# simochen/flowtrack.pytorch

Hardware: AMD Instinct MI355X
Metric: pose crops/sec (ResNet-50 + 3-deconv head, 256x192) (higher is better)
Workload: dtype fp16; 1 GPU; ResNet-50 pose head fp16, batch 64 x 256x192 synthetic crops per GPU (BASELINE.json configs[1]); per_gpu_batch=64, resident_batches=4, parallelism=dp1: batch sharded, one process per GPU

## Files before the change

flowtrack/pytorch_amd/csrc/conv_direct.hip:

```cpp
#include <stdlib.h>

#include <type_traits>

#include "ft_common.h"
#include "conv_wstat.h"

namespace ft {
namespace {

struct CdParams {
  const char* x;
  const char* x2;
  const char* res;
  char* y;
  const char* ws;
  const float* scale;
  const float* shift;
  int M;
  int nc1, nc2;
  int x_cstride, x_coff;
  int HqWq, Wq;
  int x2_hi, x2_wi, x2_cstride, x2_coff, x2_stride;
  int y_cstride, y_coff, res_cstride, res_coff;
  int Cout, act;
  float slope;
  int npt, ncb;
  unsigned x_bytes, x2_bytes, y_bytes, res_bytes, ws_bytes;
  int cpt, kw, Hi, Wi, stride, pad;
  int dbg;
  int wmajor;
};

static inline int cd_wmajor(long long x_bytes, long long w_bytes, int npt, int ncb) {
  static const int mode = dev_env_int("FT_CD_WMAJOR", 0);
  if (mode != 2) return mode == 1;
  if (ncb < 8 || npt < 2) return 0;
  return 8 * x_bytes + w_bytes < x_bytes + 8 * w_bytes;
}

template <int N, int I = 0, typename F>
__device__ __forceinline__ void cd_unroll(F&& f) {
  if constexpr (I < N) {
    f(std::integral_constant<int, I>{});
    cd_unroll<N, I + 1>(f);
  }
}

#define CD_BARRIER() asm volatile("s_barrier" ::: "memory")

__host__ __device__ constexpr int cd_sigma(int r) { return 16 * ((r >> 2) & 1) + 4 * (r >> 3) + (r & 3); }

template <int CPR>
__device__ __forceinline__ int cd_key(int row) { return CPR < 16 ? ((row >> 1) & (CPR - 1)) : (row & 15); }

#ifndef FT_CD_WSLOTS
#define FT_CD_WSLOTS 3
#endif
template <int KSPLIT>
struct CdGeom {
  static constexpr int MT = 3, BP = 96;
  static constexpr int BN = KSPLIT == 1 ? 256 : 64;
  static constexpr int CHUNK_K = KSPLIT == 1 ? 64 : 256;
  static constexpr int ROWB = CHUNK_K * 2;
  static constexpr int XB = BP * ROWB;
  static constexpr int LX = XB / 1024 / 4;
  static constexpr int WCHUNK = 4 * 8 * 1024;
  static constexpr int STG_ROWB = BN * 2;
  static constexpr int RING = 3 * XB;
  static constexpr int PART = KSPLIT == 1 ? 0 : 4 * 6 * 4096;
  static constexpr int LDS_BYTES = (RING > PART + BP * STG_ROWB ? RING : PART + BP * STG_ROWB) + 2 * BN * 4;
  static_assert(LDS_BYTES <= 163840, "LDS map");
};

template <int KSPLIT, bool HAS_RES, int NCH, bool TAPS = false>
__global__ __launch_bounds__(256, 1) void conv_direct_kernel(const CdParams p) {
#if defined(__HIP_DEVICE_COMPILE__)
  using G = CdGeom<KSPLIT>;
  constexpr int MT = G::MT, BP = G::BP, BN = G::BN, ROWB = G::ROWB, XB = G::XB, LX = G::LX;
  constexpr int TAB = G::LDS_BYTES - 2 * BN * 4;
  extern __shared__ __attribute__((aligned(16))) char smem[];
  typedef __attribute__((address_space(3))) void* lds_ptr;
  using c0 = std::integral_constant<int, 0>;
  using c1 = std::integral_constant<int, 1>;
  using c2 = std::integral_constant<int, 2>;
  const int tid = threadIdx.x, lane = tid & 63;
  const int wave = __builtin_amdgcn_readfirstlane(tid >> 6);
  const int l31 = lane & 31, lhi = lane >> 5;

  int logical;
  {
    const int total = p.npt * p.ncb;
    const int b = blockIdx.x;
    const int q = total >> 3, r = total & 7, xcd = b & 7, loc = b >> 3;
    logical = (xcd < r ? xcd * (q + 1) : r * (q + 1) + (xcd - r) * q) + loc;
  }
  const int cb = p.wmajor ? logical / p.npt : logical % p.ncb, pt = p.wmajor ? logical % p.npt : logical / p.ncb;
  const int m0 = pt * BP;
  const int nchunk = NCH > 0 ? NCH : p.nc1 + p.nc2;

  const __amdgpu_buffer_rsrc_t rsrc_x = __builtin_amdgcn_make_buffer_rsrc(const_cast<char*>(p.x), 0, p.x_bytes, 0x00020000);
  const __amdgpu_buffer_rsrc_t rsrc_x2 = __builtin_amdgcn_make_buffer_rsrc(const_cast<char*>(p.nc2 ? p.x2 : p.x), 0, p.nc2 ? p.x2_bytes : p.x_bytes, 0x00020000);
  const __amdgpu_buffer_rsrc_t rsrc_y = __builtin_amdgcn_make_buffer_rsrc(p.y, 0, p.y_bytes, 0x00020000);
  const __amdgpu_buffer_rsrc_t rsrc_w = __builtin_amdgcn_make_buffer_rsrc(const_cast<char*>(p.ws), 0, p.ws_bytes, 0x00020000);
  constexpr unsigned kOOB = 0x80000000u;

  constexpr int CPR = ROWB / 16;
  constexpr int RPL = 64 / CPR;
  unsigned x_voff[LX], x2_voff[TAPS ? 1 : LX];
  int x_tmask[TAPS ? LX : 1];
#pragma unroll
  for (int t = 0; t < LX; ++t) {
    const int row = (t * 4 + wave) * RPL + lane / CPR, pos = lane % CPR;
    const int m = m0 + row;
    const unsigned swz = (unsigned)((pos ^ cd_key<CPR>(row)) << 4);
    unsigned v = kOOB, v2 = kOOB;
    if constexpr (TAPS) {
      int mk = 0;
      if (m < p.M) {
        const int n = m / p.HqWq, rem = m - n * p.HqWq, oy = rem / p.Wq, ox = rem - oy * p.Wq;
        const int iy0 = oy * p.stride - p.pad, ix0 = ox * p.stride - p.pad;
        v = (unsigned)((((n * p.Hi + iy0) * p.Wi + ix0) * p.x_cstride + p.x_coff) * 2) + swz;
        const int ntap = p.nc1 / p.cpt;
        for (int tp = 0; tp < ntap; ++tp) {
          const int ky = tp / p.kw, kx = tp - ky * p.kw;
          if ((unsigned)(iy0 + ky) < (unsigned)p.Hi && (unsigned)(ix0 + kx) < (unsigned)p.Wi) mk |= 1 << tp;
        }
      }
      x_tmask[t] = mk;
      x_voff[t] = v;
      continue;
    }
    if (m < p.M) {
      v = (unsigned)((m * p.x_cstride + p.x_coff) * 2) + swz;
      if (p.nc2) {
        const int n = m / p.HqWq, rem = m - n * p.HqWq, qy = rem / p.Wq, qx = rem - qy * p.Wq;
        v2 = (unsigned)((((n * p.x2_hi + qy * p.x2_stride) * p.x2_wi + qx * p.x2_stride) * p.x2_cstride + p.x2_coff) * 2) + swz;
      }
    }
    x_voff[t] = v;
    x2_voff[TAPS ? 0 : t] = v2;
  }
  auto issue_x = [&](int c, int buf) {
    char* dst = smem + buf * XB;
    if constexpr (TAPS) {
      const int tap = c / p.cpt, cc = c - tap * p.cpt;
      const int ky = tap / p.kw, kx = tap - ky * p.kw;
      const unsigned delta = (unsigned)(((ky * p.Wi + kx) * p.x_cstride) * 2 + cc * ROWB);
#pragma unroll
      for (int t = 0; t < LX; ++t)
        __builtin_amdgcn_raw_ptr_buffer_load_lds(rsrc_x, (lds_ptr)(dst + (t * 4 + wave) * 1024), 16,
                                                 ((x_tmask[t] >> tap) & 1) ? x_voff[t] + delta : kOOB, 0, 0, 0);
    } else if (c < p.nc1) {
#pragma unroll
      for (int t = 0; t < LX; ++t)
        __builtin_amdgcn_raw_ptr_buffer_load_lds(rsrc_x, (lds_ptr)(dst + (t * 4 + wave) * 1024), 16, x_voff[t], c * ROWB, 0, 0);
    } else {
#pragma unroll
      for (int t = 0; t < LX; ++t)
        __builtin_amdgcn_raw_ptr_buffer_load_lds(rsrc_x2, (lds_ptr)(dst + (t * 4 + wave) * 1024), 16, x2_voff[t], (c - p.nc1) * ROWB, 0, 0);
    }
  };
  const unsigned lane16 = (unsigned)lane * 16u;
  constexpr int WS = NCH > 0 ? FT_CD_WSLOTS : 3;
  uint4_t areg[WS][4][2];
  auto load_a = [&](auto slotc, int c) {
    constexpr int SL = decltype(slotc)::value;
    const int base = c < nchunk ? ((cb * nchunk + c) * 4 + wave) * 8192 : 0x7fff0000;
#pragma unroll
    for (int kk = 0; kk < 4; ++kk)
#pragma unroll
      for (int i = 0; i < 2; ++i)
        areg[SL][kk][i] = __builtin_amdgcn_raw_buffer_load_b128(rsrc_w, lane16, base + (kk * 2 + i) * 1024, 0);
  };

  if (tid < BN / 4) {
    const float4_t one = {1.f, 1.f, 1.f, 1.f}, zero = {0.f, 0.f, 0.f, 0.f};
    const int ch = cb * BN + tid * 4;
    reinterpret_cast<float4_t*>(smem + TAB)[tid] = p.scale ? *reinterpret_cast<const float4_t*>(p.scale + ch) : one;
    reinterpret_cast<float4_t*>(smem + TAB + BN * 4)[tid] = p.shift ? *reinterpret_cast<const float4_t*>(p.shift + ch) : zero;
  }
  constexpr int NTILE = 2 * MT;
  const int wtile0 = KSPLIT == 1 ? 2 * wave : 0;
  uint4_t rres[HAS_RES ? (KSPLIT == 1 ? NTILE : 2) : 1][2];
  if constexpr (HAS_RES) {
    const __amdgpu_buffer_rsrc_t rsrc_r = __builtin_amdgcn_make_buffer_rsrc(const_cast<char*>(p.res), 0, p.res_bytes, 0x00020000);
    if constexpr (KSPLIT == 1) {
#pragma unroll
      for (int i = 0; i < 2; ++i)
#pragma unroll
        for (int j = 0; j < MT; ++j) {
          const int m = m0 + j * 32 + l31;
          const unsigned v = m < p.M ? (unsigned)((m * p.res_cstride + p.res_coff + cb * BN + (wtile0 + i) * 32 + 16 * lhi) * 2) : kOOB;
#pragma unroll
          for (int h = 0; h < 2; ++h) rres[i * MT + j][h] = __builtin_amdgcn_raw_buffer_load_b128(rsrc_r, v, h * 16, 0);
        }
    } else {
#pragma unroll
      for (int k = 0; k < 2; ++k) {
        const int tl = wave + 4 * k, i = tl / MT, j = tl - i * MT;
        const int m = m0 + j * 32 + l31;
        const unsigned v = (tl < NTILE && m < p.M) ? (unsigned)((m * p.res_cstride + p.res_coff + cb * BN + i * 32 + 16 * lhi) * 2) : kOOB;
#pragma unroll
        for (int h = 0; h < 2; ++h) rres[k][h] = __builtin_amdgcn_raw_buffer_load_b128(rsrc_r, v, h * 16, 0);
      }
    }
  }

  unsigned long long ts[8] = {0, 0, 0, 0, 0, 0, 0, 0};
#define CD_TS(i) do { if (p.dbg & 32) ts[i] = __builtin_amdgcn_s_memtime(); } while (0)
  CD_TS(0);
  issue_x(0, 0);
  issue_x(1, 1);
  issue_x(2, 2);
  cd_unroll<WS - 1>([&](auto sc) { load_a(sc, decltype(sc)::value); });

  float16_t acc[2][MT];
#pragma unroll
  for (int i = 0; i < 2; ++i)
#pragma unroll
    for (int j = 0; j < MT; ++j)
#pragma unroll
      for (int r = 0; r < 16; ++r) acc[i][j][r] = 0.f;
  int b_off[MT];
#pragma unroll
  for (int j = 0; j < MT; ++j) {
    const int row = j * 32 + l31;
    const int s0 = KSPLIT == 1 ? 0 : 4 * wave;
    b_off[j] = row * ROWB + ((((s0 * 2 + lhi) ^ cd_key<CPR>(row))) << 4);
  }
  uint4_t fx[2][MT];
// ... 11 lines not shown
      for (int j = 0; j < MT; ++j)
        acc[i][j] = __builtin_amdgcn_mfma_f32_32x32x16_f16(__builtin_bit_cast(half8_t, areg[SL][kk][i]), __builtin_bit_cast(half8_t, fx[S][j]),
                                                           acc[i][j], 0, 0, 0);
  };
  auto issue_x_dummy = [&](int buf) {
    char* dst = smem + buf * XB;
#pragma unroll
    for (int t = 0; t < LX; ++t)
      __builtin_amdgcn_raw_ptr_buffer_load_lds(rsrc_x, (lds_ptr)(dst + (t * 4 + wave) * 1024), 16, kOOB, 0, 0, 0);
  };
  auto chunk = [&](auto slotc, auto wslotc, int c) {
    constexpr int SL = decltype(slotc)::value, WL = decltype(wslotc)::value;
    using slot = std::integral_constant<int, WL>;
    load_a(std::integral_constant<int, (WL + WS - 1) % WS>{}, c + WS - 1);
    ldx(c1{}, SL, 1);
    mma(c0{}, slot{}, std::integral_constant<int, 0>{});
    ldx(c0{}, SL, 2);
    mma(c1{}, slot{}, std::integral_constant<int, 1>{});
    ldx(c1{}, SL, 3);
    mma(c0{}, slot{}, std::integral_constant<int, 2>{});
    if (c + 1 < nchunk) {
      asm volatile("s_waitcnt vmcnt(%0) lgkmcnt(0)" ::"n"(LX + 8 * (WS - 2)) : "memory");
      CD_BARRIER();
      if (c + 3 < nchunk) issue_x(c + 3, SL);
      else issue_x_dummy(SL);
      ldx(c0{}, (SL + 1) % 3, 0);
    }
    mma(c1{}, slot{}, std::integral_constant<int, 3>{});
  };

  asm volatile("s_waitcnt vmcnt(%0) lgkmcnt(0)" ::"n"(2 * LX + 8 * (WS - 1)) : "memory");
  CD_BARRIER();
  CD_TS(1);
  ldx(c0{}, 0, 0);
  if constexpr (NCH > 0) {
    cd_unroll<NCH>([&](auto cc) {
      constexpr int c = decltype(cc)::value;
      chunk(std::integral_constant<int, c % 3>{}, std::integral_constant<int, c % WS>{}, c);
    });
  } else {
    for (int c = 0; c < nchunk; c += 3) {
      chunk(c0{}, c0{}, c);
      if (c + 1 < nchunk) chunk(c1{}, c1{}, c + 1);
      if (c + 2 < nchunk) chunk(c2{}, c2{}, c + 2);
    }
  }
  CD_TS(2);
  asm volatile("s_waitcnt vmcnt(0) lgkmcnt(0)" ::: "memory");
  CD_BARRIER();
  CD_TS(3);

  const float* tsc = reinterpret_cast<const float*>(smem + TAB);
  const float* tsh = tsc + BN;
  constexpr int SCPR = G::STG_ROWB / 16;
  constexpr int SMASK = SCPR < 16 ? SCPR - 1 : 15;
  char* stg = smem + G::PART;
  const float act_k = p.act == FT_ACT_RELU ? 0.f : (p.act == FT_ACT_LEAKY ? p.slope : 1.f);
  auto finish_tile = [&](const float16_t& a, int i, int j, const uint4_t* rr) {
    const int ch = i * 32 + 16 * lhi;
    const int row = j * 32 + l31;
    float4_t sc[4], sh[4];
#pragma unroll
    for (int g4 = 0; g4 < 4; ++g4) {
      sc[g4] = *reinterpret_cast<const float4_t*>(tsc + ch + g4 * 4);
      sh[g4] = *reinterpret_cast<const float4_t*>(tsh + ch + g4 * 4);
    }
    half8_t o[2];
#pragma unroll
    for (int h = 0; h < 2; ++h) {
      half8_t rs;
      if constexpr (HAS_RES) rs = __builtin_bit_cast(half8_t, rr[h]);
#pragma unroll
      for (int e = 0; e < 8; ++e) {
        const int r = h * 8 + e;
        float v = a[r] * sc[r >> 2][r & 3] + sh[r >> 2][r & 3];
        if constexpr (HAS_RES) v += (float)rs[e];
        o[h][e] = (half_t)act_mul(v, act_k);
      }
      *reinterpret_cast<half8_t*>(stg + row * G::STG_ROWB + ((((ch >> 3) + h) ^ (row & SMASK)) << 4)) = o[h];
    }
  };
  if constexpr (KSPLIT == 1) {
#pragma unroll
    for (int i = 0; i < 2; ++i)
#pragma unroll
      for (int j = 0; j < MT; ++j) finish_tile(acc[i][j], wtile0 + i, j, HAS_RES ? rres[i * MT + j] : nullptr);
  } else {
    float4_t* part = reinterpret_cast<float4_t*>(smem);
#pragma unroll
    for (int i = 0; i < 2; ++i)
#pragma unroll
      for (int j = 0; j < MT; ++j)
#pragma unroll
        for (int g4 = 0; g4 < 4; ++g4) {
          const float4_t v = {acc[i][j][4 * g4], acc[i][j][4 * g4 + 1], acc[i][j][4 * g4 + 2], acc[i][j][4 * g4 + 3]};
          part[((wave * NTILE + i * MT + j) * 4 + g4) * 64 + lane] = v;
        }
    asm volatile("s_waitcnt lgkmcnt(0)" ::: "memory");
    CD_BARRIER();
#pragma unroll
    for (int k = 0; k < 2; ++k) {
      const int tl = wave + 4 * k;
      if (tl < NTILE) {
        float16_t sum;
#pragma unroll
        for (int g4 = 0; g4 < 4; ++g4) {
// ... 872 lines not shown
template <int MT, int NH>
static int c3s2_launch(const C3Params& p, hipStream_t s) {
  auto k = conv3x3s2_direct_kernel<MT, NH>;
  constexpr int lds = 131072 + 512 + 2 * 64 * 4 + MT * 32 * 128;
  FT_RAISE_LDS(k, lds);
  hipLaunchKernelGGL(k, dim3(p.npt * p.ncb), dim3(256), lds, s, p);
  FT_LAUNCH_CHECK("conv3x3s2_direct_kernel");
  return FT_OK;
}

template <int MT, int SPT, int TT = MT>
static int c3_launch(const C3Params& p, hipStream_t s) {
  auto k = conv3x3_direct_kernel<MT, SPT, TT>;
  constexpr int lds = 131072 + SPT * 512 + 2 * 64 * 4 + MT * 32 * 128;
  static bool attr_done[64] = {};
  int dev = 0;
  FT_HIP_CHECK(hipGetDevice(&dev));
  if (dev < 0 || dev >= 64 || !attr_done[dev]) {
    FT_HIP_CHECK(hipFuncSetAttribute(reinterpret_cast<const void*>(k), hipFuncAttributeMaxDynamicSharedMemorySize, lds));
    if (dev >= 0 && dev < 64) attr_done[dev] = true;
  }
  hipLaunchKernelGGL(k, dim3(p.npt * p.ncb), dim3(256), lds, s, p);
  FT_LAUNCH_CHECK("conv3x3_direct_kernel");
  return FT_OK;
}

template <int KSPLIT>
__global__ __launch_bounds__(256) void cd_pack_kernel(const half_t* __restrict__ w, uint4_t* __restrict__ out, int nchunk, int ncb,
                                                      int kpad, int cout_pad) {
  using G = CdGeom<KSPLIT>;
  const int idx = blockIdx.x * 256 + threadIdx.x;
  const int total = ncb * nchunk * (G::WCHUNK / 16);
  if (idx >= total) return;
  const int lane = idx & 63;
  int f = idx >> 6;
  const int i = f & 1; f >>= 1;
  const int kk = f & 3; f >>= 2;
  const int wv = f & 3; f >>= 2;
  const int c = f % nchunk, cb = f / nchunk;
  const int l31 = lane & 31, lhi = lane >> 5;
  int co, k;
  if (KSPLIT == 1) {
    co = cb * 256 + (2 * wv + i) * 32 + cd_sigma(l31);
    k = c * 64 + kk * 16 + 8 * lhi;
  } else {
    co = cb * 64 + i * 32 + cd_sigma(l31);
    k = c * 256 + (4 * wv + kk) * 16 + 8 * lhi;
  }
  uint4_t v = {0u, 0u, 0u, 0u};
  if (co < cout_pad && k < kpad) v = *reinterpret_cast<const uint4_t*>(w + (size_t)co * kpad + k);
  out[idx] = v;
}


struct CsParams {
  const char* x;
  char* y;
  const char* ws;
  const float* scale;
  const float* shift;
  int M, ntiles;
  int x_cstride, x_coff, y_cstride, y_coff;
  int Cout, act;
  float slope;
  unsigned x_bytes, y_bytes, ws_bytes;
};

template <int NS, int WC, int WP, int CT, int PT>
__global__ __launch_bounds__(64 * WC * WP, 1) void conv1x1_stream_kernel(const CsParams p) {
#if defined(__HIP_DEVICE_COMPILE__)
  constexpr int NW = WC * WP, BP = WP * PT * 32, BN = WC * CT * 32, ROWB = NS * 32, SLOTB = BP * ROWB, LX = SLOTB / 1024 / NW;
  constexpr int RPL = 1024 / ROWB, CPR = ROWB / 16;
  constexpr int NST = CT * PT * 2;
  static_assert(LX * NW * 1024 == SLOTB && 2 * SLOTB <= 160 * 1024 && RPL >= 1, "shape");
  extern __shared__ __attribute__((aligned(16))) char smem[];
  typedef __attribute__((address_space(3))) void* lds_ptr;
  const int tid = threadIdx.x, lane = tid & 63;
  const int wave = __builtin_amdgcn_readfirstlane(tid >> 6);
  const int wc = wave % WC, wp = wave / WC;
  const int l31 = lane & 31, lhi = lane >> 5;
  const int cb = blockIdx.y;
  const __amdgpu_buffer_rsrc_t rsrc_x = __builtin_amdgcn_make_buffer_rsrc(const_cast<char*>(p.x), 0, p.x_bytes, 0x00020000);
  const __amdgpu_buffer_rsrc_t rsrc_y = __builtin_amdgcn_make_buffer_rsrc(p.y, 0, p.y_bytes, 0x00020000);
  const __amdgpu_buffer_rsrc_t rsrc_w = __builtin_amdgcn_make_buffer_rsrc(const_cast<char*>(p.ws), 0, p.ws_bytes, 0x00020000);
  constexpr unsigned kOOB = 0x80000000u;

  uint4_t a[CT][NS];
#pragma unroll
  for (int i = 0; i < CT; ++i)
#pragma unroll
    for (int s = 0; s < NS; ++s)
      a[i][s] = __builtin_amdgcn_raw_buffer_load_b128(rsrc_w, (unsigned)lane * 16u, ((cb * (BN / 32) + wc * CT + i) * NS + s) * 1024, 0);
  float4_t sc[CT][4], sh[CT][4];
#pragma unroll
  for (int i = 0; i < CT; ++i)
#pragma unroll
    for (int g4 = 0; g4 < 4; ++g4) {
      const int ch = cb * BN + (wc * CT + i) * 32 + 16 * lhi + 4 * g4;
      const float4_t one = {1.f, 1.f, 1.f, 1.f}, zero = {0.f, 0.f, 0.f, 0.f};
      sc[i][g4] = p.scale ? *reinterpret_cast<const float4_t*>(p.scale + ch) : one;
      sh[i][g4] = p.shift ? *reinterpret_cast<const float4_t*>(p.shift + ch) : zero;
    }
  const float act_k = p.act == FT_ACT_RELU ? 0.f : (p.act == FT_ACT_LEAKY ? p.slope : 1.f);

  int l_row[LX];
  unsigned l_off[LX];
// ... 82 lines not shown
  const int lane = idx & 63;
  const int f = idx >> 6;
  const int sl = f % ns, tl = f / ns;
  const int co = tl * 32 + cd_sigma(lane & 31), k = sl * 16 + 8 * (lane >> 5);
  uint4_t v = {0u, 0u, 0u, 0u};
  if (co < cout_pad && k < kpad) v = *reinterpret_cast<const uint4_t*>(w + (size_t)co * kpad + k);
  out[idx] = v;
}

struct CdPlan {
  int ksplit;
  int nc1, nc2, npt, ncb;
};

static int cd_plan(const ft_conv_desc* d, CdPlan* out) {
  if (!d) return FT_ERR_INVALID_ARG;
  if (d->act == FT_ACT_LEAKY && !(d->slope >= 0.f && d->slope <= 1.f)) return FT_ERR_UNSUPPORTED;
  if (d->dtype != FT_F16 || d->transposed) return FT_ERR_UNSUPPORTED;
  const bool taps = d->kh != 1 || d->kw != 1;
  if (taps) {
    if (d->kh != 3 || d->kw != 3 || d->pad != 1 || (d->stride != 1 && d->stride != 2) || d->x2_cin || d->has_residual) return FT_ERR_UNSUPPORTED;
    if (d->Ho != (d->Hi + 2 - 3) / d->stride + 1 || d->Wo != (d->Wi + 2 - 3) / d->stride + 1) return FT_ERR_INVALID_ARG;
  } else if (d->stride != 1 || d->pad != 0) return FT_ERR_UNSUPPORTED;
  if (d->tail_cout || d->pool || d->x_wpitch || d->out_layout != FT_LAYOUT_NHWC) return FT_ERR_UNSUPPORTED;
  if (d->N <= 0 || d->Hi <= 0 || d->Wi <= 0 || (!taps && (d->Ho != d->Hi || d->Wo != d->Wi))) return FT_ERR_UNSUPPORTED;
  if (d->x_coff % 8 || d->x_cstride % 8 || d->y_coff % 8 || d->y_cstride % 8 || d->Cout % 64) return FT_ERR_UNSUPPORTED;
  if (d->x_cstride < d->x_coff + d->Cin || d->y_cstride < d->y_coff + d->Cout) return FT_ERR_INVALID_ARG;
  if (d->has_residual && (d->x2_cin || d->res_coff % 8 || d->res_cstride % 8)) return FT_ERR_UNSUPPORTED;
  if (d->x2_cin && (d->x2_coff % 8 || d->x2_cstride % 8 || d->x2_stride < 1 || d->Ho != (d->x2_hi - 1) / d->x2_stride + 1 ||
                    d->Wo != (d->x2_wi - 1) / d->x2_stride + 1)) return FT_ERR_UNSUPPORTED;
  const long long M = (long long)d->N * d->Ho * d->Wo;
  const long long lim = 1LL << 31;
  if ((long long)d->N * d->Hi * d->Wi * d->x_cstride * 2 >= lim || M * d->y_cstride * 2 >= lim || (d->has_residual && M * d->res_cstride * 2 >= lim) ||
      (d->x2_cin && (long long)d->N * d->x2_hi * d->x2_wi * d->x2_cstride * 2 >= lim)) return FT_ERR_UNSUPPORTED;
  static const int cs_mode = dev_env_int("FT_CD_STATIONARY", 1);
  const bool cs256 = d->Cin == 256 && d->Cout % 128 == 0 && M > 65536, cs512 = cs_mode == 2 && d->Cin == 512 && d->Cout == 256 && M >= 32768;
  if (!taps && cs_mode != 0 && !d->x2_cin && !d->has_residual && (cs256 || cs512)) {
    const int bp = cs256 ? 128 : 64;
    *out = CdPlan{0, d->Cin / 64, 0, (int)((M + bp - 1) / bp), cs256 ? d->Cout / 128 : 1};
    return FT_OK;
  }
  if (!taps && M > 65536) return FT_ERR_UNSUPPORTED;
  const int npt = (int)((M + 95) / 96);
  const bool a_ok = d->Cout % 256 == 0 && d->Cin % 64 == 0 && d->x2_cin % 64 == 0;
  const bool b_ok = d->Cin % 256 == 0 && d->x2_cin % 256 == 0;
  if (!a_ok && !b_ok) return FT_ERR_UNSUPPORTED;
  int ks = a_ok ? 1 : 4;
  if (a_ok && b_ok && (long long)npt * (d->Cout / 256) < 160 && d->Cout <= 512) ks = 4;
  const int ck = ks == 1 ? 64 : 256;
  *out = CdPlan{ks, d->kh * d->kw * (d->Cin / ck), d->x2_cin / ck, npt, d->Cout / (ks == 1 ? 256 : 64)};
  return FT_OK;
}

template <int KSPLIT, bool HAS_RES, int NCH, bool TAPS = false>
static int cd_launch(const CdParams& p, hipStream_t s) {
  auto k = conv_direct_kernel<KSPLIT, HAS_RES, NCH, TAPS>;
  constexpr int lds = CdGeom<KSPLIT>::LDS_BYTES;
  static_assert(lds <= 163840, "LDS map");
  static bool attr_done[64] = {};
  int dev = 0;
  FT_HIP_CHECK(hipGetDevice(&dev));
  if (dev < 0 || dev >= 64 || !attr_done[dev]) {
    FT_HIP_CHECK(hipFuncSetAttribute(reinterpret_cast<const void*>(k), hipFuncAttributeMaxDynamicSharedMemorySize, lds));
    if (dev >= 0 && dev < 64) attr_done[dev] = true;
  }
  hipLaunchKernelGGL(k, dim3(p.npt * p.ncb), dim3(256), lds, s, p);
  FT_LAUNCH_CHECK("conv_direct_kernel");
  return FT_OK;
}

template <int KSPLIT>
static int cd_dispatch_taps(const CdParams& p, hipStream_t s) {
  if (KSPLIT == 1) {
    switch (p.nc1) {
      case 36: return cd_launch<KSPLIT, false, 36, true>(p, s);
      case 72: return cd_launch<KSPLIT, false, 72, true>(p, s);
      default: return cd_launch<KSPLIT, false, 0, true>(p, s);
    }
  }
  switch (p.nc1) {
    case 9: return cd_launch<KSPLIT, false, 9, true>(p, s);
    case 18: return cd_launch<KSPLIT, false, 18, true>(p, s);
    default: return cd_launch<KSPLIT, false, 0, true>(p, s);
  }
}

template <int KSPLIT, bool HAS_RES>
static int cd_dispatch(const CdParams& p, hipStream_t s) {
  const int n = p.nc1 + p.nc2;
  if (KSPLIT == 1) {
    switch (n) {
      case 4: return cd_launch<KSPLIT, HAS_RES, 4>(p, s);
      case 6: return cd_launch<KSPLIT, HAS_RES, 6>(p, s);
      case 8: return cd_launch<KSPLIT, HAS_RES, 8>(p, s);
      case 12: return cd_launch<KSPLIT, HAS_RES, 12>(p, s);
      case 16: return cd_launch<KSPLIT, HAS_RES, 16>(p, s);
      case 24: return cd_launch<KSPLIT, HAS_RES, 24>(p, s);
      default: return cd_launch<KSPLIT, HAS_RES, 0>(p, s);
    }
  }
  switch (n) {
    case 2: return cd_launch<KSPLIT, HAS_RES, 2>(p, s);
    case 4: return cd_launch<KSPLIT, HAS_RES, 4>(p, s);
    case 8: return cd_launch<KSPLIT, HAS_RES, 8>(p, s);
    default: return cd_launch<KSPLIT, HAS_RES, 0>(p, s);
  }
}

}
}

extern "C" int ft_conv_direct_supported(const ft_conv_desc* d) {
  ft::CdPlan pl;
  ft::C3Plan p3;
  ft::WsPlan pw;
  if (d && d->kh == 5) return ft::ws_plan(d, &pw);
  if (d && d->kh == 3 && ft::c3_plan(d, &p3) == FT_OK) return FT_OK;
  return ft::cd_plan(d, &pl);
}

extern "C" int ft_conv_direct_stream_id(const ft_conv_desc* d) {
  ft::CdPlan pl;
  ft::C3Plan p3;
  ft::WsPlan pw;
  if (d && d->kh == 5) return ft::ws_plan(d, &pw) == FT_OK ? (0x50000000 | pw.ncg) : -1;
  if (d && d->kh == 3 && ft::c3_plan(d, &p3) == FT_OK) return 0x40000000 | (p3.stride == 2 ? (p3.ipw == 2 ? 0x30000000 : 0x10000000) : 0) | (p3.ncb << 8) | p3.spt;
  if (ft::cd_plan(d, &pl) != FT_OK) return -1;
  return ((pl.ksplit + 1) << 24) | ((pl.nc1 + pl.nc2) << 12) | pl.ncb;
}

extern "C" long long ft_conv_direct_weight_bytes(const ft_conv_desc* d) {
  ft::CdPlan pl;
  ft::C3Plan p3;
  ft::WsPlan pw;
  if (d && d->kh == 5) return ft::ws_plan(d, &pw) == FT_OK ? ft::ws_weight_bytes(pw) : 0;
  if (d && d->kh == 3 && ft::c3_plan(d, &p3) == FT_OK) return (long long)p3.ncb * 4 * 9 * p3.spt * 8192;
  if (ft::cd_plan(d, &pl) != FT_OK) return 0;
  if (pl.ksplit == 0) return (long long)d->Cout * d->Cin * 2;
  return (long long)pl.ncb * (pl.nc1 + pl.nc2) * 32768;
}

extern "C" int ft_conv_direct_pack(const ft_conv_desc* d, const void* w_packed, int kpad, int cout_pad, void* wstream, ft_stream_t stream) {
  using namespace ft;
  C3Plan p3;
  if (d && d->kh == 5) {
    WsPlan pw;
    const int st = ws_plan(d, &pw);
    return st != FT_OK ? st : ws_pack(d, pw, w_packed, kpad, cout_pad, wstream, as_stream(stream));
  }
  if (d && d->kh == 3 && c3_plan(d, &p3) == FT_OK) {
    if (!w_packed || !wstream || kpad < 9 * d->Cin || cout_pad < d->Cout) return FT_ERR_INVALID_ARG;
    const int total = p3.ncb * 4 * 9 * p3.spt * 512;
    const dim3 pg(ceil_div(total, 256));
    const half_t* wsrc = static_cast<const half_t*>(w_packed);
    uint4_t* wdst = static_cast<uint4_t*>(wstream);
    if (p3.stride == 2 && p3.ipw == 2) hipLaunchKernelGGL(c3s2p_pack_kernel, pg, dim3(256), 0, as_stream(stream), wsrc, wdst, p3.ncb, kpad, cout_pad);
    else if (p3.stride == 2) hipLaunchKernelGGL(c3s2_pack_kernel<2>, pg, dim3(256), 0, as_stream(stream), wsrc, wdst, p3.ncb, kpad, cout_pad);
    else if (p3.spt == 4) hipLaunchKernelGGL(c3_pack_kernel<4>, pg, dim3(256), 0, as_stream(stream), wsrc, wdst, p3.ncb, kpad, cout_pad);
    else hipLaunchKernelGGL(c3_pack_kernel<2>, pg, dim3(256), 0, as_stream(stream), wsrc, wdst, p3.ncb, kpad, cout_pad);
    FT_LAUNCH_CHECK("c3_pack_kernel");
    return FT_OK;
  }
  CdPlan pl;
  const int st = cd_plan(d, &pl);
  if (st != FT_OK) return st;
  if (!w_packed || !wstream || kpad < d->kh * d->kw * d->Cin + d->x2_cin || cout_pad < d->Cout) return FT_ERR_INVALID_ARG;
  const int nchunk = pl.nc1 + pl.nc2;
  const int total = pl.ncb * nchunk * 2048;
  hipStream_t s = as_stream(stream);
  if (pl.ksplit == 0) {
    const int ntile = d->Cout / 32, ns = d->Cin / 16;
    hipLaunchKernelGGL(cs_pack_kernel, dim3(ceil_div(ntile * ns * 64, 256)), dim3(256), 0, s, static_cast<const half_t*>(w_packed),
                       static_cast<uint4_t*>(wstream), ntile, ns, kpad, cout_pad);
    FT_LAUNCH_CHECK("cs_pack_kernel");
    return FT_OK;
  }
  if (pl.ksplit == 1)
    hipLaunchKernelGGL(cd_pack_kernel<1>, dim3(ceil_div(total, 256)), dim3(256), 0, s, static_cast<const half_t*>(w_packed),
                       static_cast<uint4_t*>(wstream), nchunk, pl.ncb, kpad, cout_pad);
  else
    hipLaunchKernelGGL(cd_pack_kernel<4>, dim3(ceil_div(total, 256)), dim3(256), 0, s, static_cast<const half_t*>(w_packed),
                       static_cast<uint4_t*>(wstream), nchunk, pl.ncb, kpad, cout_pad);
  FT_LAUNCH_CHECK("cd_pack_kernel");
  return FT_OK;
}

extern "C" int ft_conv_direct_fwd(const ft_conv_desc* d, const void* x, const void* wstream, const float* scale, const float* shift,
                                  const void* residual, void* y, ft_stream_t stream) {
  using namespace ft;
  C3Plan p3;
  if (d && d->kh == 5) {
    WsPlan pw;
    const int st = ws_plan(d, &pw);
    return st != FT_OK ? st : ws_launch(d, pw, x, wstream, scale, shift, y, as_stream(stream));
  }
  if (d && d->kh == 3 && c3_plan(d, &p3) == FT_OK) {
    if (!x || !wstream || !y) return FT_ERR_INVALID_ARG;
    C3Params q{};
    q.x = static_cast<const char*>(x);
    q.y = static_cast<char*>(y);
    q.ws = static_cast<const char*>(wstream);
    q.scale = scale;
    q.shift = shift;
    q.HW = d->Hi * d->Wi; q.W = d->Wi; q.H = d->Hi; q.ipw = p3.ipw;
    q.Ho = p3.stride == 2 ? d->Ho : 0; q.Wo = p3.stride == 2 ? d->Wo : 0;
    q.strip_rows = p3.strip_rows; q.nstrips = p3.nstrips;
    q.M = p3.stride == 2 ? d->N * d->Ho * d->Wo : d->N * q.HW;
    q.x_cstride = d->x_cstride; q.x_coff = d->x_coff; q.y_cstride = d->y_cstride; q.y_coff = d->y_coff;
    q.Cout = d->Cout; q.act = d->act; q.slope = d->slope;
    q.npt = p3.npt; q.ncb = p3.ncb;
    q.x_bytes = (unsigned)((size_t)d->N * q.HW * d->x_cstride * 2);
    q.y_bytes = (unsigned)((size_t)q.M * d->y_cstride * 2);
    q.ws_bytes = (unsigned)ft_conv_direct_weight_bytes(d);
    q.wmajor = cd_wmajor((long long)d->N * q.HW * d->Cin * 2, q.ws_bytes, q.npt, q.ncb);
    if (p3.stride == 2 && p3.ipw == 2) {
      const int nld = (2 * q.HW * 256 + 4095) / 4096;
      if (p3.mt <= 2) return nld <= 16 ? c3s2p_launch<2, 16>(q, as_stream(stream)) : c3s2p_launch<2, 32>(q, as_stream(stream));
      return nld <= 24 ? c3s2p_launch<3, 24>(q, as_stream(stream)) : c3s2p_launch<3, 32>(q, as_stream(stream));
    }
    if (p3.stride == 2) return p3.mt == 1 ? c3s2_launch<1, 2>(q, as_stream(stream)) : c3s2_launch<2, 2>(q, as_stream(stream));
    if (p3.strip_rows) return c3_launch<3, 2, 4>(q, as_stream(stream));
    if (p3.spt == 4) return c3_launch<2, 4>(q, as_stream(stream));
    return p3.mt == 3 ? c3_launch<3, 2>(q, as_stream(stream)) : c3_launch<4, 2>(q, as_stream(stream));
  }
  CdPlan pl;
  const int st = cd_plan(d, &pl);
  if (st != FT_OK) return st;
  if (!x || !wstream || !y || ((d->has_residual || d->x2_cin) && !residual)) return FT_ERR_INVALID_ARG;
  if (pl.ksplit == 0) {
    CsParams q{};
    q.x = static_cast<const char*>(x);
    q.y = static_cast<char*>(y);
    q.ws = static_cast<const char*>(wstream);
    q.scale = scale;
    q.shift = shift;
    q.M = d->N * d->Ho * d->Wo;
    q.ntiles = pl.npt;
    q.x_cstride = d->x_cstride; q.x_coff = d->x_coff; q.y_cstride = d->y_cstride; q.y_coff = d->y_coff;
    q.Cout = d->Cout; q.act = d->act; q.slope = d->slope;
    q.x_bytes = (unsigned)((size_t)q.M * d->x_cstride * 2);
    q.y_bytes = (unsigned)((size_t)q.M * d->y_cstride * 2);
    q.ws_bytes = (unsigned)ft_conv_direct_weight_bytes(d);
    constexpr int lds = 2 * 65536;
// ... 51 lines not shown
```

flowtrack/pytorch_amd/hip_ops.py:

```python
from __future__ import annotations

import ctypes
import functools
import json
import os
import sys
from dataclasses import dataclass
from typing import List, Optional, Sequence, Tuple

import torch

from . import _lib
from ._lib import (FT_ACT_LEAKY, FT_ACT_NONE, FT_ACT_RELU, FT_LAYOUT_NCHW_F32, FT_LAYOUT_NHWC,
                   ConvDesc, ConvGeometry, FlowtrackHipError, check)

ACT_CODES = {None: FT_ACT_NONE, "none": FT_ACT_NONE, "relu": FT_ACT_RELU, "leaky": FT_ACT_LEAKY}


def require_gpu(device: torch.device) -> None:
    if device.type != "cuda" or not torch.cuda.is_available():
        raise FlowtrackHipError(
            "the flowtrack HIP path needs a ROCm GPU (model.cuda()); there is no CPU fallback — "
            "use oracle/ for CPU reference results")

# ... 659 lines not shown
                raise FlowtrackHipError(f"{self.label}: x_nchw must be the contiguous fp32 [N, Cin, H, W] input of a pooled stem")
        elif x.t.device.type == "meta":
            raise FlowtrackHipError(f"{self.label}: a geometry-only input view needs x_nchw")
        Ho, Wo = self.out_hw(x.H, x.W)
        d = ConvDesc()
        d.dtype = self.code
        d.N, d.Hi, d.Wi = x.N, x.H, x.W
        d.Cin, d.x_cstride, d.x_coff = self.cin, x.cstride, x.coff
        if x.rowpacked:
            d.x_lpad, d.x_wpitch = x.lpad, x.wpitch
        d.Cout, d.kh, d.kw = self.cout, self.k, self.k
        d.stride, d.pad, d.transposed = self.stride, self.pad, int(self.transposed)
        d.Ho, d.Wo = Ho, Wo
        out_c = self.tail_cout or self.cout
        if pool:
            if Ho % 2 or Wo % 2 or not isinstance(y, ActView) or residual is not None or self.tail_cout:
                raise FlowtrackHipError(f"{self.label}: the fused max-pool needs an even conv output and a plain NHWC result")
            d.pool = 1
        yH, yW = (Ho // 2, Wo // 2) if pool else (Ho, Wo)
        if isinstance(y, ActView):
            if (y.N, y.H, y.W) != (x.N, yH, yW) or y.C != out_c or y.t.dtype != self.dtype:
                raise FlowtrackHipError(f"{self.label}: output view mismatch {tuple(y.t.shape)} C={y.C}")
            d.y_cstride, d.y_coff, d.out_layout = y.cstride, y.coff, FT_LAYOUT_NHWC
            yt = y.t
        else:
            if tuple(y.shape) != (x.N, out_c, Ho, Wo) or y.dtype != torch.float32 or not y.is_contiguous():
                raise FlowtrackHipError(f"{self.label}: NCHW output must be contiguous fp32 {(x.N, out_c, Ho, Wo)}")
            d.y_cstride, d.y_coff, d.out_layout = 0, 0, FT_LAYOUT_NCHW_F32
            yt = y
        res_ptr = None
        if residual is not None:
            if (residual.N, residual.H, residual.W) != (x.N, Ho, Wo) or residual.C != self.cout:
                raise FlowtrackHipError(f"{self.label}: residual view mismatch")
            d.has_residual, d.res_cstride, d.res_coff = 1, residual.cstride, residual.coff
            res_ptr = residual.t.data_ptr()
        d.act, d.slope = self.act, self.slope
        if self.tail_cout:
            if residual is not None:
                raise FlowtrackHipError(f"{self.label}: a fused tail excludes a residual input")
            d.tail_cout = self.tail_cout
            res_ptr = self._tail.data_ptr()
        x_ptr, x_keep = x.t.data_ptr() if x_nchw is None else x_nchw.data_ptr(), x.t if x_nchw is None else x_nchw
        if x_nchw is not None:
            d.x_nchw_f32 = 1
        w, _, scale, shift = self._packed_for(d)
        if shift_n is not None:
            d.shift_nstride = self.cout
            if self.lib.ft_conv_shift_nstride_supported(ctypes.byref(d)) != 0:
                raise FlowtrackHipError(f"{self.label}: per-sample shift is not supported for this layer / shape")
            shift = shift_n(scale, shift)
            if tuple(shift.shape) != (x.N, self.cout) or shift.dtype != torch.float32 or not shift.is_contiguous():
                raise FlowtrackHipError(f"{self.label}: per-sample shift must be contiguous fp32 {(x.N, self.cout)}")
        flops = float(self.lib.ft_conv_flops(ctypes.byref(d)))
        ws = _direct_stream(self, d, w, x.t.device) if (self.k in (1, 3, 5) and isinstance(y, ActView) and not self.tail_cout and not pool) else None
        if ws is not None:
            dd = ConvDesc.from_buffer_copy(d)
            prog.begin_choice("conv|" + _desc_key(d))
            prog.option("direct")
            prog.flops += flops
            prog.conv_records.append((self.label, len(prog.calls), flops, dd))
            prog.add("ft_conv_direct_fwd", ctypes.byref(dd), x.t.data_ptr(), ws.data_ptr(),
                     scale.data_ptr() if scale is not None else None, shift.data_ptr() if shift is not None else None, res_ptr,
                     yt.data_ptr(), keep=(dd, x.t, yt, ws, scale, shift, residual.t if residual is not None else None))
            prog.option("igemm")
        self._record_igemm(prog, d, x, w, scale, shift, res_ptr, yt, residual, flops, x_ptr, x_keep)
        if ws is not None:
            prog.end_choice()

    def _record_igemm(self, prog: Program, d: ConvDesc, x: ActView, w, scale, shift, res_ptr, yt, residual, flops: float,
                      x_ptr=None, x_keep=None) -> None:
        x_ptr = x.t.data_ptr() if x_ptr is None else x_ptr
        x_keep = x.t if x_keep is None else x_keep
        prog.flops += flops
        prog.conv_records.append((self.label, len(prog.calls), flops, d))
        if prog._side:
            prog.add("ft_conv2d_fwd", ctypes.byref(d), x_ptr, w.data_ptr(),
                     scale.data_ptr() if scale is not None else None,
                     shift.data_ptr() if shift is not None else None, res_ptr, yt.data_ptr(),
                     keep=(d, x_keep, yt, w, scale, shift, residual.t if residual is not None else None, self._tail))
            return
        prog.need_workspace(self.lib.ft_conv_workspace_bytes(ctypes.byref(d)))
        prog.add("ft_conv2d_fwd_ws", ctypes.byref(d), x_ptr, w.data_ptr(),
                 scale.data_ptr() if scale is not None else None,
                 shift.data_ptr() if shift is not None else None, res_ptr, yt.data_ptr(), prog._ws_ptr, prog._ws_size,
                 keep=(d, x_keep, yt, w, scale, shift, residual.t if residual is not None else None, self._tail))


CONV_DIRECT = os.environ.get("FT_CONV_DIRECT", "1") != "0"
CONV_DIRECT_MAX_PIXELS = int(os.environ.get("FT_CONV_DIRECT_MAX_PIXELS", "65536"))


def _direct_stream(owner, d: ConvDesc, w: torch.Tensor, device) -> Optional[torch.Tensor]:
    lib = _lib.load()
    wstat = d.kh == 5 and d.Cin == 64 and d.stride == 2 and not d.x2_cin
    if not CONV_DIRECT or d.dtype != _lib.FT_F16 or (d.Cin + d.x2_cin < 256 and not wstat) or (d.kh == 5 and not wstat):
        return None
    if not wstat and d.N * d.Ho * d.Wo > CONV_DIRECT_MAX_PIXELS and not (CONV_DIRECT_MAX_PIXELS >= 65536 and d.kh == 1 and d.Cin in (256, 512)
                                                          and not d.x2_cin and not d.has_residual):
        return None
    if lib.ft_conv_direct_supported(ctypes.byref(d)) != 0:
        return None
    sid = int(lib.ft_conv_direct_stream_id(ctypes.byref(d)))
    if sid < 0:
        return None
    key = ("direct", sid, w.data_ptr())
    hit = owner._packed.get(key)
    if hit is None:
# ... 516 lines not shown
```

Before: 59090 crops/s.

## Add direct-stream kernel path for stride-2 4x4 transposed convolutions

```diff
diff --git a/flowtrack/pytorch_amd/csrc/conv_direct.hip b/flowtrack/pytorch_amd/csrc/conv_direct.hip
--- a/flowtrack/pytorch_amd/csrc/conv_direct.hip
+++ b/flowtrack/pytorch_amd/csrc/conv_direct.hip
@@ -72,9 +72,14 @@
   static_assert(LDS_BYTES <= 163840, "LDS map");
 };
 
-template <int KSPLIT, bool HAS_RES, int NCH, bool TAPS = false>
+constexpr int cd_transposed(int nch) { return -1 - nch; }
+
+template <int KSPLIT, bool HAS_RES, int NCHF, bool TAPS = false>
 __global__ __launch_bounds__(256, 1) void conv_direct_kernel(const CdParams p) {
 #if defined(__HIP_DEVICE_COMPILE__)
+  constexpr bool DECONV = NCHF < 0;
+  constexpr int NCH = DECONV ? -1 - NCHF : NCHF;
+  static_assert(!DECONV || (KSPLIT == 1 && !HAS_RES && !TAPS), "the transposed form is the plain N-tile-256 walk");
   using G = CdGeom<KSPLIT>;
   constexpr int MT = G::MT, BP = G::BP, BN = G::BN, ROWB = G::ROWB, XB = G::XB, LX = G::LX;
   constexpr int TAB = G::LDS_BYTES - 2 * BN * 4;
@@ -95,7 +100,8 @@
     logical = (xcd < r ? xcd * (q + 1) : r * (q + 1) + (xcd - r) * q) + loc;
   }
   const int cb = p.wmajor ? logical / p.npt : logical % p.ncb, pt = p.wmajor ? logical % p.npt : logical / p.ncb;
-  const int m0 = pt * BP;
+  const int tile_rows = DECONV ? p.cpt * p.HqWq : BP;
+  const int m0 = pt * tile_rows;
   const int nchunk = NCH > 0 ? NCH : p.nc1 + p.nc2;
 
   const __amdgpu_buffer_rsrc_t rsrc_x = __builtin_amdgcn_make_buffer_rsrc(const_cast<char*>(p.x), 0, p.x_bytes, 0x00020000);
@@ -130,7 +136,7 @@
       x_voff[t] = v;
       continue;
     }
-    if (m < p.M) {
+    if (m < p.M && (!DECONV || row < tile_rows)) {
       v = (unsigned)((m * p.x_cstride + p.x_coff) * 2) + swz;
       if (p.nc2) {
         const int n = m / p.HqWq, rem = m - n * p.HqWq, qy = rem / p.Wq, qx = rem - qy * p.Wq;
@@ -173,9 +179,9 @@
         areg[SL][kk][i] = __builtin_amdgcn_raw_buffer_load_b128(rsrc_w, lane16, base + (kk * 2 + i) * 1024, 0);
   };
 
-  if (tid < BN / 4) {
+  if (tid < (DECONV ? 16 : BN) / 4) {
     const float4_t one = {1.f, 1.f, 1.f, 1.f}, zero = {0.f, 0.f, 0.f, 0.f};
-    const int ch = cb * BN + tid * 4;
+    const int ch = cb * (DECONV ? 16 : BN) + tid * 4;
     reinterpret_cast<float4_t*>(smem + TAB)[tid] = p.scale ? *reinterpret_cast<const float4_t*>(p.scale + ch) : one;
     reinterpret_cast<float4_t*>(smem + TAB + BN * 4)[tid] = p.shift ? *reinterpret_cast<const float4_t*>(p.shift + ch) : zero;
   }
@@ -293,6 +299,77 @@
 
   const float* tsc = reinterpret_cast<const float*>(smem + TAB);
   const float* tsh = tsc + BN;
+  if constexpr (DECONV) {
+    static_assert(BP * 512 <= TAB, "LDS map");
+    const float act_k = p.act == FT_ACT_RELU ? 0.f : (p.act == FT_ACT_LEAKY ? p.slope : 1.f);
+    const int HW = p.HqWq, Wo = 2 * p.Wi, OHW2 = 2 * HW;
+    const int nitems = p.cpt * OHW2 * 2;
+#pragma unroll
+    for (int pass = 0; pass < 2; ++pass) {
+      if (pass) CD_BARRIER();
+      if ((wave & 1) != pass) {
+#pragma unroll
+        for (int i = 0; i < 2; ++i)
+#pragma unroll
+          for (int j = 0; j < MT; ++j) {
+            const int row = j * 32 + l31, slot = (wave >> 1) * 4 + 2 * i + lhi;
+#pragma unroll
+            for (int g4 = 0; g4 < 4; ++g4) {
+              const float4_t v = {acc[i][j][4 * g4], acc[i][j][4 * g4 + 1], acc[i][j][4 * g4 + 2], acc[i][j][4 * g4 + 3]};
+              *reinterpret_cast<float4_t*>(smem + row * 512 + (((slot * 4 + g4) ^ (row & 15)) << 4)) = v;
+            }
+          }
+      }
+      asm volatile("s_waitcnt lgkmcnt(0)" ::: "memory");
+      CD_BARRIER();
+      if (pass == 0) CD_TS(4);
+#pragma unroll
+      for (int k = 0; k < 2; ++k) {
+        const int idx = tid + 256 * k;
+        if (idx >= nitems) continue;
+        const int h = idx & 1, q = idx >> 1;
+        const int img = q / OHW2, rem = q - img * OHW2, oyh = rem / Wo, ox = rem - oyh * Wo, oy = 2 * oyh + pass;
+        float4_t s0 = {0.f, 0.f, 0.f, 0.f}, s1 = {0.f, 0.f, 0.f, 0.f};
+#pragma unroll
+        for (int a = 0; a < 2; ++a) {
+          const int iy = oyh + pass - a;
+#pragma unroll
+          for (int b = 0; b < 2; ++b) {
+            const int kx = ((ox + 1) & 1) + 2 * b, ix = (ox + 1 - kx) >> 1;
+            if ((unsigned)iy < (unsigned)p.Hi && (unsigned)ix < (unsigned)p.Wi) {
+              const int row = img * HW + iy * p.Wi + ix, pos = (a * 4 + kx) * 4 + 2 * h;
+              const char* rp = smem + row * 512;
+              s0 += *reinterpret_cast<const float4_t*>(rp + ((pos ^ (row & 15)) << 4));
+              s1 += *reinterpret_cast<const float4_t*>(rp + (((pos + 1) ^ (row & 15)) << 4));
+            }
+          }
+        }
+        const float4_t sc0 = *reinterpret_cast<const float4_t*>(tsc + 8 * h), sc1 = *reinterpret_cast<const float4_t*>(tsc + 8 * h + 4);
+        const float4_t sh0 = *reinterpret_cast<const float4_t*>(tsh + 8 * h), sh1 = *reinterpret_cast<const float4_t*>(tsh + 8 * h + 4);
+        half8_t o;
+#pragma unroll
+        for (int e = 0; e < 4; ++e) {
+          o[e] = (half_t)act_mul(s0[e] * sc0[e] + sh0[e], act_k);
+          o[4 + e] = (half_t)act_mul(s1[e] * sc1[e] + sh1[e], act_k);
+        }
+        const int mi = m0 + img * HW;
+        const unsigned voff = mi < p.M ? (unsigned)(((mi * 4 + oy * Wo + ox) * p.y_cstride + p.y_coff + cb * 16 + 8 * h) * 2) : kOOB;
+        if (p.dbg & 64) __builtin_amdgcn_raw_buffer_store_b128(__builtin_bit_cast(uint4_t, o), rsrc_y, voff, 0, 16);
+        else __builtin_amdgcn_raw_buffer_store_b128(__builtin_bit_cast(uint4_t, o), rsrc_y, voff, 0, 0);
+      }
+    }
+    if (p.dbg & 32) {
+      ts[5] = __builtin_amdgcn_s_memtime();
+      asm volatile("s_waitcnt vmcnt(0)" ::: "memory");
+      ts[6] = __builtin_amdgcn_s_memtime();
+      if (tid < 2 && m0 < p.M) {
+        unsigned long long* o = reinterpret_cast<unsigned long long*>(p.y + ((size_t)(m0 * 4 + tid) * p.y_cstride + p.y_coff + cb * 16) * 2);
+#pragma unroll
+        for (int i = 0; i < 4; ++i) o[i] = ts[4 * tid + i];
+      }
+    }
+    return;
+  }
   constexpr int SCPR = G::STG_ROWB / 16;
   constexpr int SMASK = SCPR < 16 ? SCPR - 1 : 15;
   char* stg = smem + G::PART;
@@ -1271,6 +1348,22 @@
   out[idx] = v;
 }
 
+__global__ __launch_bounds__(256) void cdt_pack_kernel(const half_t* __restrict__ w, uint4_t* __restrict__ out, int nchunk, int ncb,
+                                                       int kpad, int cout_pad) {
+  const int idx = blockIdx.x * 256 + threadIdx.x;
+  if (idx >= ncb * nchunk * 2048) return;
+  const int lane = idx & 63;
+  int f = idx >> 6;
+  const int i = f & 1; f >>= 1;
+  const int kk = f & 3; f >>= 2;
+  const int wv = f & 3; f >>= 2;
+  const int c = f % nchunk, cb = f / nchunk;
+  const int col = (2 * wv + i) * 32 + cd_sigma(lane & 31);
+  const int ky = col >> 6, kx = (col >> 4) & 3, co = cb * 16 + (col & 15);
+  const int phase = ((ky & 1) ? 0 : 2) + ((kx & 1) ? 0 : 1), tap = (ky >> 1) * 2 + (kx >> 1);
+  const int k = tap * (nchunk * 64) + c * 64 + kk * 16 + 8 * (lane >> 5);
+  out[idx] = *reinterpret_cast<const uint4_t*>(w + ((size_t)phase * cout_pad + co) * kpad + k);
+}
 
 struct CsParams {
   const char* x;
@@ -1459,6 +1552,36 @@
   return FT_OK;
 }
 
+static int cdt_plan(const ft_conv_desc* d, CdPlan* out) {
+  if (!d) return FT_ERR_INVALID_ARG;
+  if (d->act == FT_ACT_LEAKY && !(d->slope >= 0.f && d->slope <= 1.f)) return FT_ERR_UNSUPPORTED;
+  if (d->dtype != FT_F16 || d->transposed != 1 || d->kh != 4 || d->kw != 4 || d->stride != 2 || d->pad != 1) return FT_ERR_UNSUPPORTED;
+  if (d->has_residual || d->x2_cin || d->tail_cout || d->pool || d->x_wpitch || d->shift_nstride || d->x_nchw_f32 ||
+      d->out_layout != FT_LAYOUT_NHWC) return FT_ERR_UNSUPPORTED;
+  if (d->N <= 0 || d->Hi <= 0 || d->Wi <= 0 || d->Cin <= 0 || d->Cout <= 0) return FT_ERR_UNSUPPORTED;
+  if (d->Ho != 2 * d->Hi || d->Wo != 2 * d->Wi) return FT_ERR_INVALID_ARG;
+  if ((long long)d->Hi * d->Wi > 96 || d->Cin % 64 || d->Cout % 16) return FT_ERR_UNSUPPORTED;
+  if (d->x_coff % 8 || d->x_cstride % 8 || d->y_coff % 8 || d->y_cstride % 8) return FT_ERR_UNSUPPORTED;
+  if (d->x_cstride < d->x_coff + d->Cin || d->y_cstride < d->y_coff + d->Cout) return FT_ERR_INVALID_ARG;
+  const long long lim = 1LL << 31;
+  if ((long long)d->N * d->Hi * d->Wi * d->x_cstride * 2 >= lim || (long long)d->N * d->Ho * d->Wo * d->y_cstride * 2 >= lim ||
+      32LL * d->Cin * d->Cout >= lim) return FT_ERR_UNSUPPORTED;
+  const int ipw = 96 / (d->Hi * d->Wi);
+  *out = CdPlan{1, d->Cin / 64, 0, (d->N + ipw - 1) / ipw, d->Cout / 16};
+  return FT_OK;
+}
+
+template <int NCH>
+static int cdt_launch(const CdParams& p, hipStream_t s) {
+  auto k = conv_direct_kernel<1, false, cd_transposed(NCH)>;
+  constexpr int lds = CdGeom<1>::LDS_BYTES;
+  static_assert(lds <= 163840, "LDS map");
+  FT_RAISE_LDS(k, lds);
+  hipLaunchKernelGGL(k, dim3(p.npt * p.ncb), dim3(256), lds, s, p);
+  FT_LAUNCH_CHECK("conv_direct_kernel (transposed)");
+  return FT_OK;
+}
+
 template <int KSPLIT, bool HAS_RES, int NCH, bool TAPS = false>
 static int cd_launch(const CdParams& p, hipStream_t s) {
   auto k = conv_direct_kernel<KSPLIT, HAS_RES, NCH, TAPS>;
@@ -1521,6 +1644,7 @@
   ft::CdPlan pl;
   ft::C3Plan p3;
   ft::WsPlan pw;
+  if (d && d->transposed) return ft::cdt_plan(d, &pl);
   if (d && d->kh == 5) return ft::ws_plan(d, &pw);
   if (d && d->kh == 3 && ft::c3_plan(d, &p3) == FT_OK) return FT_OK;
   return ft::cd_plan(d, &pl);
@@ -1530,6 +1654,7 @@
   ft::CdPlan pl;
   ft::C3Plan p3;
   ft::WsPlan pw;
+  if (d && d->transposed) return ft::cdt_plan(d, &pl) == FT_OK ? (0x60000000 | (pl.nc1 << 12) | pl.ncb) : -1;
   if (d && d->kh == 5) return ft::ws_plan(d, &pw) == FT_OK ? (0x50000000 | pw.ncg) : -1;
   if (d && d->kh == 3 && ft::c3_plan(d, &p3) == FT_OK) return 0x40000000 | (p3.stride == 2 ? (p3.ipw == 2 ? 0x30000000 : 0x10000000) : 0) | (p3.ncb << 8) | p3.spt;
   if (ft::cd_plan(d, &pl) != FT_OK) return -1;
@@ -1540,6 +1665,7 @@
   ft::CdPlan pl;
   ft::C3Plan p3;
   ft::WsPlan pw;
+  if (d && d->transposed) return ft::cdt_plan(d, &pl) == FT_OK ? (long long)pl.ncb * pl.nc1 * 32768 : 0;
   if (d && d->kh == 5) return ft::ws_plan(d, &pw) == FT_OK ? ft::ws_weight_bytes(pw) : 0;
   if (d && d->kh == 3 && ft::c3_plan(d, &p3) == FT_OK) return (long long)p3.ncb * 4 * 9 * p3.spt * 8192;
   if (ft::cd_plan(d, &pl) != FT_OK) return 0;
@@ -1550,6 +1676,16 @@
 extern "C" int ft_conv_direct_pack(const ft_conv_desc* d, const void* w_packed, int kpad, int cout_pad, void* wstream, ft_stream_t stream) {
   using namespace ft;
   C3Plan p3;
+  if (d && d->transposed) {
+    CdPlan pt;
+    const int st = cdt_plan(d, &pt);
+    if (st != FT_OK) return st;
+    if (!w_packed || !wstream || kpad < 4 * d->Cin || cout_pad < d->Cout) return FT_ERR_INVALID_ARG;
+    hipLaunchKernelGGL(cdt_pack_kernel, dim3(pt.ncb * pt.nc1 * 8), dim3(256), 0, as_stream(stream), static_cast<const half_t*>(w_packed),
+                       static_cast<uint4_t*>(wstream), pt.nc1, pt.ncb, kpad, cout_pad);
+    FT_LAUNCH_CHECK("cdt_pack_kernel");
+    return FT_OK;
+  }
   if (d && d->kh == 5) {
     WsPlan pw;
     const int st = ws_plan(d, &pw);
@@ -1596,6 +1732,37 @@
                                   const void* residual, void* y, ft_stream_t stream) {
   using namespace ft;
   C3Plan p3;
+  if (d && d->transposed) {
+    CdPlan pt;
+    const int st = cdt_plan(d, &pt);
+    if (st != FT_OK) return st;
+    if (!x || !wstream || !y) return FT_ERR_INVALID_ARG;
+    CdParams p{};
+    p.x = static_cast<const char*>(x);
+    p.y = static_cast<char*>(y);
+    p.ws = static_cast<const char*>(wstream);
+    p.scale = scale;
+    p.shift = shift;
+    p.M = d->N * d->Hi * d->Wi;
+    p.nc1 = pt.nc1; p.npt = pt.npt; p.ncb = pt.ncb;
+    p.x_cstride = d->x_cstride; p.x_coff = d->x_coff;
+    p.HqWq = d->Hi * d->Wi; p.Wq = d->Wi; p.Hi = d->Hi; p.Wi = d->Wi;
+    p.cpt = 96 / p.HqWq;
+    p.y_cstride = d->y_cstride; p.y_coff = d->y_coff;
+    p.Cout = d->Cout; p.act = d->act; p.slope = d->slope;
+    p.x_bytes = (unsigned)((size_t)p.M * d->x_cstride * 2);
+    p.y_bytes = (unsigned)((size_t)p.M * 4 * d->y_cstride * 2);
+    p.ws_bytes = (unsigned)((size_t)pt.ncb * pt.nc1 * 32768);
+    static const int dbg = dev_env_int("FT_CD_DBG", 0);
+    p.dbg = dbg;
+    p.wmajor = cd_wmajor((long long)p.M * d->Cin * 2, p.ws_bytes, p.npt, p.ncb);
+    hipStream_t s = as_stream(stream);
+    switch (pt.nc1) {
+      case 4: return cdt_launch<4>(p, s);
+      case 32: return cdt_launch<32>(p, s);
+      default: return cdt_launch<0>(p, s);
+    }
+  }
   if (d && d->kh == 5) {
     WsPlan pw;
     const int st = ws_plan(d, &pw);
diff --git a/flowtrack/pytorch_amd/hip_ops.py b/flowtrack/pytorch_amd/hip_ops.py
--- a/flowtrack/pytorch_amd/hip_ops.py
+++ b/flowtrack/pytorch_amd/hip_ops.py
@@ -735,7 +735,7 @@
             if tuple(shift.shape) != (x.N, self.cout) or shift.dtype != torch.float32 or not shift.is_contiguous():
                 raise FlowtrackHipError(f"{self.label}: per-sample shift must be contiguous fp32 {(x.N, self.cout)}")
         flops = float(self.lib.ft_conv_flops(ctypes.byref(d)))
-        ws = _direct_stream(self, d, w, x.t.device) if (self.k in (1, 3, 5) and isinstance(y, ActView) and not self.tail_cout and not pool) else None
+        ws = _direct_stream(self, d, w, x.t.device) if ((self.k in (1, 3, 5) or self.transposed) and isinstance(y, ActView) and not self.tail_cout and not pool) else None
         if ws is not None:
             dd = ConvDesc.from_buffer_copy(d)
             prog.begin_choice("conv|" + _desc_key(d))
```

Result: faster. 60270 crops/s (median of 6 runs) (+2.0%).
